# sshaoshuai/PointRCNN

Hardware: AMD Instinct MI355X
Metric: KITTI frames/sec, RPN inference end-to-end (16384 pts/frame, bs32 per GPU) (higher is better)
Workload: dtype f32 via split-bf16x6 MFMA (every fp32 operand cut exactly into 3 bf16 pieces, 6 bf16 MFMA products per fp32 product, fp32 accumulate: fp32-grade, measured error 2.9e-7 of sum|x||w| vs 3.0e-7 for the fp32-MFMA kernel; hoisted grouped layers on the split kernel too, unhoisted grouped first layers (xyz; 1 GPU; Full RPN PointNet++ backbone (4 SA-MSG + 4 FP) + cls/reg heads, tools/cfgs/default.yaml, 16384 pts/frame, batch 32 per GPU, random-init weights, eval-mode BN; frames_per_gpu=32, npoints=16384, parallelism=frames sharded, dp1, launch=hipGraph replay, streams=20, hw_queues=4, proposal_layer=normal, clouds=uniform, group_dedup=True, roi_dedup=True

## Files before the change

### include/prcnn_pointops.h

```cpp
#ifndef PRCNN_POINTOPS_H
#define PRCNN_POINTOPS_H

#include <stddef.h>
#include <stdint.h>

#ifdef __cplusplus
extern "C" {
#endif

typedef void* prcnn_stream_t;

#define PRCNN_OK 0
#define PRCNN_EINVAL (-1)
#define PRCNN_EHIP (-2)
#define PRCNN_EUNSUPPORTED (-3)

int prcnn_abi_version(void);
const char* prcnn_last_error(void);
const char* prcnn_build_id(void);
int prcnn_switches_reload(void);
int prcnn_switch_get(const char* name, int* set, long* num);


int prcnn_fps(const float* xyz, int B, int N, int npoint, float* tmp, int32_t* idx, prcnn_stream_t stream);

int prcnn_fps_status(void);

#define PRCNN_FPS_ORDER_CANONICAL 0
#define PRCNN_FPS_ORDER_UPSTREAM 1
int prcnn_fps_order(const float* xyz, int B, int N, int npoint, int order, float* tmp, int32_t* idx, prcnn_stream_t stream);

#define PRCNN_ARITH_CANONICAL 0
#define PRCNN_ARITH_UPSTREAM 1
int prcnn_fps_mode(const float* xyz, int B, int N, int npoint, int order, int arith, float* tmp, int32_t* idx, prcnn_stream_t stream);
int prcnn_ball_query_arith(const float* xyz, const float* new_xyz, int B, int N, int M, float radius, int nsample, int arith,
                           int32_t* idx, prcnn_stream_t stream);
int prcnn_three_nn_arith(const float* unknown, const float* known, int B, int n, int m, int arith, float* dist2, int32_t* idx,
                         prcnn_stream_t stream);

int prcnn_gather(const float* feat, const int32_t* idx, int B, int C, int N, int M, float* out, prcnn_stream_t stream);
int prcnn_gather_grad(const float* grad_out, const int32_t* idx, int B, int C, int N, int M, float* grad_feat,
                      prcnn_stream_t stream);

int prcnn_gather_rows(const float* in_cl, int ld_in, const int32_t* idx, int B, int N, int M, int C, float* out,
                      prcnn_stream_t stream);

int prcnn_ball_query(const float* xyz, const float* new_xyz, int B, int N, int M, float radius, int nsample,
                     int32_t* idx, prcnn_stream_t stream);
int prcnn_ball_query2(const float* xyz, const float* new_xyz, int B, int N, int M, float radius_a, int nsample_a,
                      int32_t* idx_a, float radius_b, int nsample_b, int32_t* idx_b, prcnn_stream_t stream);

int prcnn_group(const float* feat, const int32_t* idx, int B, int C, int N, int M, int nsample, float* out,
                prcnn_stream_t stream);
int prcnn_group_grad(const float* grad_out, const int32_t* idx, int B, int C, int N, int M, int nsample,
                     float* grad_feat, prcnn_stream_t stream);

int prcnn_three_nn(const float* unknown, const float* known, int B, int n, int m, float* dist2, int32_t* idx,
// ... 272 lines not shown
```

### pointrcnn_amd/_cabi.py

```python
import contextlib
import ctypes
import os

from . import build as _build

_P = ctypes.c_void_p
_I = ctypes.c_int
_F = ctypes.c_float
_L = ctypes.c_int64
_Z = ctypes.c_size_t
_D = ctypes.c_double



class TrainSrc(ctypes.Structure):
    _fields_ = [("mode", _I), ("rows", _L), ("K", _I),
                ("in_", _P), ("ld_in", _I), ("pro_scale", _P), ("pro_shift", _P),
                ("xyz", _P), ("new_xyz", _P), ("idx", _P), ("feat", _P), ("ld_feat", _I),
                ("B", _I), ("N", _I), ("M", _I), ("ns", _I), ("C", _I),
                ("known", _P), ("idx3", _P), ("w3", _P), ("skip", _P), ("ld_known", _I), ("ld_skip", _I),
                ("n", _I), ("m", _I), ("C2", _I), ("C1", _I),
                ("mult", _P), ("rows_dev", _P), ("norm_rows", _L), ("seg_off", _P), ("seg_cnt", _P), ("row_grp", _P), ("groups", _I)]


class TrainLayer(ctypes.Structure):
    _fields_ = [("Nout", _I), ("W", _P), ("gamma", _P), ("beta", _P), ("eps", _F), ("momentum", _F),
                ("running_mean", _P), ("running_var", _P), ("y", _P), ("cst", _P), ("ld_c", _I), ("wpack", _P), ("wpack_t", _P),
                ("dW", _P), ("dgamma", _P), ("dbeta", _P)]


class RpnLossCfg(ctypes.Structure):
    _fields_ = [("loc_scope", _D), ("loc_bin_size", _D), ("mean_size", _D * 3), ("gamma", _D), ("alpha", _D), ("loss_weight", _D * 2),
                ("num_head_bin", _I), ("xz_fine", _I), ("y_by_bin", _I), ("ry_fine", _I), ("loss_cls", _I), ("has_alpha", _I)]


class RcnnLossCfg(ctypes.Structure):
    _fields_ = [("loc_scope", _D), ("loc_bin_size", _D), ("loc_y_scope", _D), ("loc_y_bin_size", _D), ("mean_size", _D * 3), ("gamma", _D),
                ("alpha", _D), ("num_head_bin", _I), ("y_by_bin", _I), ("size_res_on_roi", _I), ("loss_cls", _I), ("has_alpha", _I)]


REQUIRED_ABI = 12

SIGNATURES = {
    "prcnn_abi_version": (_I, []),
    "prcnn_last_error": (ctypes.c_char_p, []),
    "prcnn_build_id": (ctypes.c_char_p, []),
    "prcnn_switches_reload": (_I, []),
    "prcnn_switch_get": (_I, [ctypes.c_char_p, ctypes.POINTER(_I), ctypes.POINTER(ctypes.c_long)]),
    "prcnn_fps": (_I, [_P, _I, _I, _I, _P, _P, _P]),
    "prcnn_fps_status": (_I, []),
    "prcnn_fps_order": (_I, [_P, _I, _I, _I, _I, _P, _P, _P]),
    "prcnn_fps_mode": (_I, [_P, _I, _I, _I, _I, _I, _P, _P, _P]),
    "prcnn_ball_query_arith": (_I, [_P, _P, _I, _I, _I, _F, _I, _I, _P, _P]),
    "prcnn_three_nn_arith": (_I, [_P, _P, _I, _I, _I, _I, _P, _P, _P]),
    "prcnn_rpn_labels": (_I, [_P, _P, _P, _I, _I, _I, _F, _P, _P, _P]),
    "prcnn_gt_aug_edit": (_I, [_P, _P, _P, _P, _P, _F, _P, _P, _P, _I, _I, _I, _I, _P, _P, _P, _P, _P]),
    "prcnn_corner_iou3d": (_I, [_P, _I, _P, _I, _P, _P, _P]),
    "prcnn_gt_aug_sample": (_I, [_P, _P, _P, _I, _I, _P, _P, _P, _I, _P, _I, _P, _I, _P, _P, _I, _I, ctypes.c_uint32,
                                 _P, _P, _P, _P, _P, _P, _P, _P]),
    "prcnn_host_pts_in_boxes3d": (_I, [_P, _P, _L, _L, _P]),
    "prcnn_host_roipool3d": (_I, [_P, _P, _P, _L, _L, _L, _L, _P, _P, _P]),
    "prcnn_gather": (_I, [_P, _P, _I, _I, _I, _I, _P, _P]),
    "prcnn_gather_grad": (_I, [_P, _P, _I, _I, _I, _I, _P, _P]),
    "prcnn_gather_rows": (_I, [_P, _I, _P, _I, _I, _I, _I, _P, _P]),
    "prcnn_ball_query": (_I, [_P, _P, _I, _I, _I, _F, _I, _P, _P]),
    "prcnn_ball_query2": (_I, [_P, _P, _I, _I, _I, _F, _I, _P, _F, _I, _P, _P]),
    "prcnn_group": (_I, [_P, _P, _I, _I, _I, _I, _I, _P, _P]),
    "prcnn_group_grad": (_I, [_P, _P, _I, _I, _I, _I, _I, _P, _P]),
    "prcnn_three_nn": (_I, [_P, _P, _I, _I, _I, _P, _P, _P, _P]),
    "prcnn_three_interp": (_I, [_P, _P, _P, _I, _I, _I, _I, _P, _P]),
    "prcnn_three_interp_grad": (_I, [_P, _P, _P, _I, _I, _I, _I, _P, _P, _P]),
    "prcnn_wpack_floats": (_Z, [_I, _I]),
    "prcnn_pack_weight": (_I, [_P, _I, _I, _I, _P, _P]),
    "prcnn_mlp_rows": (_I, [_P, _I, _L, _I, _P, _P, _I, _I, _P, _I, _I, _I, _P, _I, _P, _I, _P]),
    "prcnn_mlp_group": (_I, [_P, _P, _P, _P, _I, _I, _I, _I, _I, _I, _P, _P, _P, _P, _I, _I, _P, _I, _I, _I, _P, _P]),
    "prcnn_mlp_group_split": (_I, [_P, _P, _P, _P, _I, _I, _I, _I, _I, _I, _P, _P, _P, _P, _I, _P, _I, _I, _P, _I, _I, _I, _P, _P]),
    "prcnn_mlp_interp": (_I, [_P, _I, _P, _P, _P, _I, _I, _I, _I, _I, _I, _P, _P, _P, _I, _I, _P, _I, _I, _P]),
    "prcnn_mlp_rows_addinterp": (_I, [_P, _I, _I, _P, _P, _I, _I, _P, _I, _P, _P, _I, _I, _I, _P, _I, _I, _P]),
    "prcnn_wsplit_bytes": (_Z, [_I, _I]),
    "prcnn_pack_weight_split": (_I, [_P, _I, _I, _I, _P, _P]),
    "prcnn_mlp_chain_interp_split": (_I, [_P, _I, _P, _P, _I, _I, _I, _I, _P, _P, _P, _P, _I, _I, _I, _P, _I, _I, _P]),
    "prcnn_mlp_chain_rows_split": (_I, [_P, _I, _L, _I, _P, _P, _P, _P, _P, _I, _P, _I, _I, _P]),
# ... 146 lines not shown
```

### pointrcnn_amd/csrc/fps.hip

```cpp
#include "lds_sort.h"
#include "switches.h"

typedef float f32x2 __attribute__((ext_vector_type(2)));
template <int PPT> struct fvec_t { typedef float type __attribute__((ext_vector_type(PPT))); };
template <> struct fvec_t<1> { typedef float type __attribute__((ext_vector_type(2))); };

#define FPS_DPP_MAX(v, ctrl) asm volatile("s_nop 1\n\tv_max_i32_dpp %0, %0, %0 " ctrl : "+v"(v))

__device__ __forceinline__ int wave_max_i32_fused(int v) {
    FPS_DPP_MAX(v, "row_shr:1 row_mask:0xf bank_mask:0xf");
    FPS_DPP_MAX(v, "row_shr:2 row_mask:0xf bank_mask:0xf");
    FPS_DPP_MAX(v, "row_shr:4 row_mask:0xf bank_mask:0xf");
    FPS_DPP_MAX(v, "row_shr:8 row_mask:0xf bank_mask:0xf");
    FPS_DPP_MAX(v, "row_bcast:15 row_mask:0xa bank_mask:0xf");
    FPS_DPP_MAX(v, "row_bcast:31 row_mask:0xc bank_mask:0xf");
    asm volatile("s_nop 1");
    return __builtin_amdgcn_readlane(v, 63);
}
__device__ __forceinline__ int row0_max_i32_fused(int v) {
    FPS_DPP_MAX(v, "row_shr:1 row_mask:0xf bank_mask:0xf");
    FPS_DPP_MAX(v, "row_shr:2 row_mask:0xf bank_mask:0xf");
    FPS_DPP_MAX(v, "row_shr:4 row_mask:0xf bank_mask:0xf");
    FPS_DPP_MAX(v, "row_shr:8 row_mask:0xf bank_mask:0xf");
    asm volatile("s_nop 1");
// ... 76 lines not shown
                     : [best] "v"(best), [p0] "v"(pt[0]), [p1] "v"(pt[1]), [p2] "v"(pt[2]), [p3] "v"(pt[3])
                     : "vcc");
        eqbits = acc;
        return t;
    }
};

#define FPS_EQ2(pa, pb) "v_cmp_eq_f32_e64 %[sa], " pa ", %[best]\n\tv_cmp_eq_f32_e64 %[sb], " pb ", %[best]\n\t"
#define FPS_AC2 "v_addc_co_u32_e64 %[a0], vcc, %[a0], %[a0], %[sa]\n\tv_addc_co_u32_e64 %[a1], vcc, %[a1], %[a1], %[sb]\n\t"
template <class V> __device__ __forceinline__ int wave_max_eq2_16(const V& pt, float best, unsigned& eqbits) {
    int t; unsigned a0, a1; unsigned long long sa, sb, sc, sd;
    asm volatile("v_mov_b32 %[t], %[best]\n\tv_mov_b32 %[a0], 0\n\tv_mov_b32 %[a1], 0\n\t"
                 FPS_EQ2("%[p15]", "%[p7]") FPS_D1 FPS_AC2
                 FPS_EQ2("%[p14]", "%[p6]") FPS_D2 FPS_AC2
                 FPS_EQ2("%[p13]", "%[p5]") FPS_D3 FPS_AC2
                 FPS_EQ2("%[p12]", "%[p4]") FPS_D4 FPS_AC2
                 FPS_EQ2("%[p11]", "%[p3]") FPS_D5 FPS_AC2
                 FPS_EQ2("%[p10]", "%[p2]") FPS_D6 FPS_AC2
                 FPS_EQ2("%[p9]", "%[p1]")
                 "v_cmp_eq_f32_e64 %[sc], %[p8], %[best]\n\tv_cmp_eq_f32_e64 %[sd], %[p0], %[best]\n\t"
                 FPS_AC2
                 "v_addc_co_u32_e64 %[a0], vcc, %[a0], %[a0], %[sc]\n\tv_addc_co_u32_e64 %[a1], vcc, %[a1], %[a1], %[sd]\n\t"
                 : [t] "=&v"(t), [a0] "=&v"(a0), [a1] "=&v"(a1), [sa] "=&s"(sa), [sb] "=&s"(sb), [sc] "=&s"(sc), [sd] "=&s"(sd)
                 : [best] "v"(best), [p0] "v"(pt[0]), [p1] "v"(pt[1]), [p2] "v"(pt[2]), [p3] "v"(pt[3]), [p4] "v"(pt[4]), [p5] "v"(pt[5]),
                   [p6] "v"(pt[6]), [p7] "v"(pt[7]), [p8] "v"(pt[8]), [p9] "v"(pt[9]), [p10] "v"(pt[10]), [p11] "v"(pt[11]),
                   [p12] "v"(pt[12]), [p13] "v"(pt[13]), [p14] "v"(pt[14]), [p15] "v"(pt[15])
                 : "vcc");
    eqbits = (a0 << 8) | a1;
    return t;
}

template <int BLOCK, int PPT>
__global__ __launch_bounds__(BLOCK) void fps_reg_kernel(const float* __restrict__ xyz, int N, int npoint,
                                                        int32_t* __restrict__ idx_out) {
    constexpr int NW = BLOCK / 64;
    typedef typename fvec_t<PPT>::type fvec;
    __shared__ float slot[2][NW][8];

    const int b = blockIdx.x;
    const int tid = threadIdx.x;
    const int lane = tid & 63;
    const int wave = tid >> 6;
    const float* __restrict__ p = xyz + (size_t)b * N * 3;
    int32_t* __restrict__ out = idx_out + (size_t)b * npoint;

    fvec px, py, pz, pt;
#pragma unroll
    for (int i = 0; i < PPT; i++) {
        int k = tid * PPT + i;
        bool ok = k < N;
        px[i] = ok ? p[k * 3 + 0] : 0.f;
        py[i] = ok ? p[k * 3 + 1] : 0.f;
        pz[i] = ok ? p[k * 3 + 2] : 0.f;
        pt[i] = ok ? 1e10f : -1.0f;
    }
    if (tid == 0 && npoint > 0) out[0] = 0;
    float x0 = p[0], y0 = p[1], z0 = p[2];

    for (int j = 1; j < npoint; j++) {
        float best = -2.0f;
        if (PPT >= 2) {
            const f32x2 qx = {x0, x0}, qy = {y0, y0}, qz = {z0, z0};
#pragma unroll
            for (int i = 0; i + 1 < PPT; i += 2) {
                f32x2 dx = (f32x2){px[i], px[i + 1]} - qx;
                f32x2 dy = (f32x2){py[i], py[i + 1]} - qy;
                f32x2 dz = (f32x2){pz[i], pz[i + 1]} - qz;
// ... 31 lines not shown
            }
            __syncthreads();
            const float* r = slot[j & 1][lane < NW ? lane : 0];
            int v = lane < NW ? __float_as_int(r[0]) : (int)0x80000000;
            int id = __float_as_int(r[1]);
            float rx = r[2], ry = r[3], rz = r[4];
            const int gmax = row0_max_i32_fused(v);
            const int wwin = __builtin_ctzll(__ballot(v == gmax));
            gidx = __builtin_amdgcn_readlane(id, wwin);
            x0 = __int_as_float(__builtin_amdgcn_readlane(__float_as_int(rx), wwin));
            y0 = __int_as_float(__builtin_amdgcn_readlane(__float_as_int(ry), wwin));
            z0 = __int_as_float(__builtin_amdgcn_readlane(__float_as_int(rz), wwin));
        }
        if (tid == 0) out[j] = gidx;
    }
}

#define FPS_BIG 1.0e18f
#ifndef FPS_V
#define FPS_V 6
#endif
#ifndef FPS_PAIR_ASM
#define FPS_PAIR_ASM 1
#endif

__device__ __forceinline__ unsigned morton_spread6(unsigned v) {
    v &= 0x3fu;
    v = (v | (v << 8)) & 0x0000300fu;
    v = (v | (v << 4)) & 0x000030c3u;
    v = (v | (v << 2)) & 0x00009249u;
    return v;
}

__global__ __launch_bounds__(1024) void fps_sort_kernel(const float* __restrict__ xyz, int N, int NP, int32_t* __restrict__ perm) {
    extern __shared__ unsigned keys[];
    __shared__ float red[6][16];
    const int b = blockIdx.x, tid = threadIdx.x, lane = tid & 63, wave = tid >> 6, nw = blockDim.x >> 6;
    const float* __restrict__ p = xyz + (size_t)b * N * 3;
    float lo[3] = {FPS_BIG, FPS_BIG, FPS_BIG}, hi[3] = {-FPS_BIG, -FPS_BIG, -FPS_BIG};
    for (int k = tid; k < N; k += blockDim.x)
#pragma unroll
        for (int a = 0; a < 3; a++) { float v = p[k * 3 + a]; lo[a] = fminf(lo[a], v); hi[a] = fmaxf(hi[a], v); }
#pragma unroll
    for (int a = 0; a < 3; a++) {
        for (int o = 32; o > 0; o >>= 1) { lo[a] = fminf(lo[a], __shfl_xor(lo[a], o)); hi[a] = fmaxf(hi[a], __shfl_xor(hi[a], o)); }
        if (lane == 0) { red[a][wave] = lo[a]; red[3 + a][wave] = hi[a]; }
    }
    __syncthreads();
    float scale[3];
#pragma unroll
    for (int a = 0; a < 3; a++) {
        float l = red[a][0], h = red[3 + a][0];
        for (int w = 1; w < nw; w++) { l = fminf(l, red[a][w]); h = fmaxf(h, red[3 + a][w]); }
        lo[a] = l;
        scale[a] = (h > l) ? 63.0f / (h - l) : 0.f;
    }
    unsigned v[16];
    if (tid * 16 < NP) {
#pragma unroll
        for (int e = 0; e < 16; e++) {
            const int k = tid * 16 + e;
            unsigned key = ~0u;
            if (k < N) {
                unsigned qx = (unsigned)((p[k * 3 + 0] - lo[0]) * scale[0]);
                unsigned qy = (unsigned)((p[k * 3 + 1] - lo[1]) * scale[1]);
                unsigned qz = (unsigned)((p[k * 3 + 2] - lo[2]) * scale[2]);
                unsigned m = (morton_spread6(qx) << 2) | (morton_spread6(qz) << 1) | morton_spread6(qy);
// ... 50 lines not shown
}
__device__ __forceinline__ void fps_xt_publish(unsigned (*xt)[64], int cb, int wave, const fps_cand_t& c) {
    unsigned* t = xt[cb];
    t[wave] = __float_as_uint(c.x); t[16 + wave] = __float_as_uint(c.y); t[32 + wave] = __float_as_uint(c.z);
    asm volatile("ds_max_u64 %0, %1 offset:192" : : "v"((unsigned)(size_t)&t[0]), "v"(c.key) : "memory");
    if (wave == 0) *(unsigned long long*)&xt[cb == 2 ? 0 : cb + 1][48] = 0ULL;
}
__device__ __forceinline__ int fps_xt_collect(unsigned (*xt)[64], int cb, int lane, float& x0, float& y0, float& z0, int& wl) {
    const int tv = (int)xt[cb][lane];
    const unsigned klo = (unsigned)__builtin_amdgcn_readlane(tv, 48);
    wl = (int)(klo & 15u);
    x0 = __int_as_float(__builtin_amdgcn_readlane(tv, wl));
    y0 = __int_as_float(__builtin_amdgcn_readlane(tv, wl | 16));
    z0 = __int_as_float(__builtin_amdgcn_readlane(tv, wl | 32));
    return (int)(0xFFFFFFFu - (klo >> 4));
}

#ifdef PRCNN_FPS_TIMING
__device__ unsigned long long prcnn_fps_dbg[16 * 8 + 16 + 16 * 16];
PRCNN_API int prcnn_fps_timing_read(unsigned long long* host_out) {
    return hipMemcpyFromSymbol(host_out, HIP_SYMBOL(prcnn_fps_dbg), sizeof(prcnn_fps_dbg)) == hipSuccess ? 0 : -1;
}
#define FPS_T(...) __VA_ARGS__
#ifndef PRCNN_FPS_TIMING_WAVE
#define PRCNN_FPS_TIMING_WAVE -1
#endif
#define FPS_NOW(w) ((PRCNN_FPS_TIMING_WAVE < 0 || (w) == PRCNN_FPS_TIMING_WAVE) ? __builtin_readcyclecounter() : 0ULL)
#else
#define FPS_T(...)
#endif

template <int PPT>
__global__ __launch_bounds__(1024) void fps_pruned_kernel(const float* __restrict__ xyz, const int32_t* __restrict__ perm,
                                                          int N, int npoint, int32_t* __restrict__ idx_out) {
    constexpr int BLOCK = 1024, NW = 16;
    typedef typename fvec_t<PPT>::type fvec;
    FPS_XT_DECL;
    extern __shared__ int s_po[];
    __builtin_amdgcn_s_setprio(2);

    const int b = blockIdx.x, tid = threadIdx.x, lane = tid & 63, wave = tid >> 6;
    const int wave_u = __builtin_amdgcn_readfirstlane(wave);
    const float* __restrict__ p = xyz + (size_t)b * N * 3;
    const int32_t* __restrict__ pm = perm + (size_t)b * N;
    int32_t* __restrict__ out = idx_out + (size_t)b * npoint;

    fvec px, py, pz, pt;
    float lox = FPS_BIG, loy = FPS_BIG, loz = FPS_BIG, hix = -FPS_BIG, hiy = -FPS_BIG, hiz = -FPS_BIG;
#pragma unroll
    for (int i = 0; i < PPT; i++) {
        int s = tid * PPT + i;
        bool ok = s < N;
        int o = ok ? pm[s] : 0x7fffffff;
        s_po[i * BLOCK + tid] = o;
        px[i] = ok ? p[o * 3 + 0] : 0.f;
        py[i] = ok ? p[o * 3 + 1] : 0.f;
        pz[i] = ok ? p[o * 3 + 2] : 0.f;
        pt[i] = ok ? 1e10f : -1.0f;
        if (ok) {
            lox = fminf(lox, px[i]); hix = fmaxf(hix, px[i]);
            loy = fminf(loy, py[i]); hiy = fmaxf(hiy, py[i]);
            loz = fminf(loz, pz[i]); hiz = fmaxf(hiz, pz[i]);
        }
    }
    lox = wave_min_f32_fused(lox); loy = wave_min_f32_fused(loy); loz = wave_min_f32_fused(loz);
    hix = wave_max_f32_fused(hix); hiy = wave_max_f32_fused(hiy); hiz = wave_max_f32_fused(hiz);

// ... 78 lines not shown
                cy = __int_as_float(__builtin_amdgcn_readlane(__float_as_int(by), owner));
                cz = __int_as_float(__builtin_amdgcn_readlane(__float_as_int(bz), owner));
            }
            cval = wmaxf;
            first = false;
            fps_cand_set(cand, wave, cx, cy, cz, cval, corig);
            FPS_T(t_u4 += __builtin_readcyclecounter() - u3;)
            }
            __builtin_amdgcn_s_setprio(2);
        }
#if FPS_V & 2
        else __builtin_amdgcn_s_setprio(2);
#endif
        FPS_T(unsigned long long t1 = __builtin_readcyclecounter(); t_upd += t1 - t0; n_upd += update ? 1 : 0;)
        if (lane == 0) fps_xt_publish(xt, cb, wave, cand);
        __syncthreads();
        FPS_T(unsigned long long t2 = __builtin_readcyclecounter(); t_wait += t2 - t1;)
        int wwin;
        const int gorig = fps_xt_collect(xt, cb, lane, x0, y0, z0, wwin);
#if FPS_V & 2
        if ((unsigned)(wave_u - wwin + 1) <= 2u) __builtin_amdgcn_s_setprio(3);
#endif
        wprev = wwin;
        cb = cb == 2 ? 0 : cb + 1;
        if (tid == 0) out[j] = gorig;
        FPS_T(t0 = __builtin_readcyclecounter(); t_red += t0 - t2;)
    }
    FPS_T(if (b == 0 && lane == 0) { unsigned long long* d = prcnn_fps_dbg + wave * 8; d[0] = t_upd; d[1] = t_wait; d[2] = t_red; d[3] = n_upd;
                                     d[4] = __builtin_readcyclecounter() - t_begin; d[5] = t_u1; d[6] = t_u2; d[7] = t_u3; prcnn_fps_dbg[128 + wave] = t_u4; })
}

template <int PPT, int NW>
__global__ __launch_bounds__(NW * 64) void fps_slot_kernel(const float* __restrict__ xyz, const int32_t* __restrict__ perm,
                                                          int N, int npoint, int32_t* __restrict__ idx_out) {
    constexpr int BLOCK = NW * 64;
    typedef typename fvec_t<PPT>::type fvec;
    FPS_XT_DECL;
    extern __shared__ int s_po[];
    __builtin_amdgcn_s_setprio(2);

    const int b = blockIdx.x, tid = threadIdx.x, lane = tid & 63, wave = tid >> 6;
    const int wave_u = __builtin_amdgcn_readfirstlane(wave);
    const float* __restrict__ p = xyz + (size_t)b * N * 3;
    const int32_t* __restrict__ pm = perm + (size_t)b * N;
    int32_t* __restrict__ out = idx_out + (size_t)b * npoint;

    fvec px, py, pz, pt;
    float lox = FPS_BIG, loy = FPS_BIG, loz = FPS_BIG, hix = -FPS_BIG, hiy = -FPS_BIG, hiz = -FPS_BIG;
#pragma unroll
    for (int i = 0; i < PPT; i++) {
        int s = (wave * PPT + i) * 64 + lane;
        bool ok = s < N;
        int o = ok ? pm[s] : 0x7fffffff;
        s_po[i * BLOCK + tid] = o;
        px[i] = ok ? p[o * 3 + 0] : 0.f;
        py[i] = ok ? p[o * 3 + 1] : 0.f;
        pz[i] = ok ? p[o * 3 + 2] : 0.f;
        pt[i] = ok ? 1e10f : -1.0f;
        if (ok) {
            lox = fminf(lox, px[i]); hix = fmaxf(hix, px[i]);
            loy = fminf(loy, py[i]); hiy = fmaxf(hiy, py[i]);
            loz = fminf(loz, pz[i]); hiz = fmaxf(hiz, pz[i]);
        }
    }
    lox = wave_min_f32_fused(lox); loy = wave_min_f32_fused(loy); loz = wave_min_f32_fused(loz);
    hix = wave_max_f32_fused(hix); hiy = wave_max_f32_fused(hiy); hiz = wave_max_f32_fused(hiz);

// ... 136 lines not shown
        }
#if FPS_V & 2
        else __builtin_amdgcn_s_setprio(2);
#endif
        FPS_T(unsigned long long q4 = FPS_NOW(wave);)
        if (lane == 0) fps_xt_publish(xt, cb, wave, cand);
        __syncthreads();
        FPS_T(unsigned long long q5 = FPS_NOW(wave); q_pub += q5 - q4;)
        int wwin;
        const int gorig = fps_xt_collect(xt, cb, lane, x0, y0, z0, wwin);
#if FPS_V & 2
        if ((unsigned)(wave_u - wwin + 1) <= 2u) __builtin_amdgcn_s_setprio(3);
#endif
        wprev = wwin;
        cb = cb == 2 ? 0 : cb + 1;
        if (tid == 0) out[j] = gorig;
        FPS_T(q0 = FPS_NOW(wave); q_coll += q0 - q5;)
    }
    FPS_T(if (b == 0 && lane == 0) { unsigned long long* d = prcnn_fps_dbg + 144 + wave * 16; d[0] = q_test; d[1] = q_dist; d[2] = q_max; d[3] = q_search; d[4] = q_pub;
                                     d[5] = q_coll; d[6] = q_nupd; d[7] = q_npair; d[8] = FPS_NOW(wave) - q_begin; })
}

struct fps_bcand_t { float x, y, z, v, s; unsigned orig, mask; unsigned long long key; };
__device__ __forceinline__ void fps_bcand_set(fps_bcand_t& c, int wave, float cx, float cy, float cz, float cval, float csec, int corig, unsigned cmask) {
    const unsigned hi = (unsigned)__float_as_int(cval) ^ 0x80000000u;
    const unsigned o = (unsigned)min(corig, 0xFFFFFFF);
    c.x = cx; c.y = cy; c.z = cz; c.v = cval; c.s = csec; c.orig = o; c.mask = cmask; c.key = ((unsigned long long)hi << 32) | ((0xFFFFFFFu - o) << 4) | (unsigned)wave;
    asm volatile("" : "+v"(c.x), "+v"(c.y), "+v"(c.z), "+v"(c.v), "+v"(c.s), "+v"(c.orig), "+v"(c.mask), "+v"(c.key));
}
#define FPS_BT_WORDS 160

template <int PPT, int NW>
__global__ __launch_bounds__(NW * 64) void fps_batch_kernel(const float* __restrict__ xyz, const int32_t* __restrict__ perm,
                                                           int N, int npoint, int32_t* __restrict__ idx_out) {
    static_assert(NW == 16 && PPT == 16, "rows of 16 lanes = the 16 waves; 8 pair boxes");
    constexpr int BLOCK = NW * 64;
    typedef typename fvec_t<PPT>::type fvec;
    typedef float f32x4 __attribute__((ext_vector_type(4)));
    typedef unsigned u32x4 __attribute__((ext_vector_type(4)));
    __shared__ __attribute__((aligned(256))) unsigned xt[3][FPS_BT_WORDS];
    __shared__ __attribute__((aligned(32))) float wbox[16][8];
    extern __shared__ int s_po[];
    __builtin_amdgcn_s_setprio(2);

    const int b = blockIdx.x, tid = threadIdx.x, lane = tid & 63, wave = tid >> 6, l15 = lane & 15;
    const int wave_u = __builtin_amdgcn_readfirstlane(wave);
    const float* __restrict__ p = xyz + (size_t)b * N * 3;
    const int32_t* __restrict__ pm = perm + (size_t)b * N;
    int32_t* __restrict__ out = idx_out + (size_t)b * npoint;

    fvec px, py, pz, pt;
    float lox = FPS_BIG, loy = FPS_BIG, loz = FPS_BIG, hix = -FPS_BIG, hiy = -FPS_BIG, hiz = -FPS_BIG;
#pragma unroll
    for (int i = 0; i < PPT; i++) {
        int s = (wave * PPT + i) * 64 + lane;
        bool ok = s < N;
        int o = ok ? pm[s] : 0x7fffffff;
        s_po[i * BLOCK + tid] = o;
        px[i] = ok ? p[o * 3 + 0] : 0.f;
        py[i] = ok ? p[o * 3 + 1] : 0.f;
        pz[i] = ok ? p[o * 3 + 2] : 0.f;
        pt[i] = ok ? 1e10f : -1.0f;
        if (ok) {
            lox = fminf(lox, px[i]); hix = fmaxf(hix, px[i]);
            loy = fminf(loy, py[i]); hiy = fmaxf(hiy, py[i]);
            loz = fminf(loz, pz[i]); hiz = fmaxf(hiz, pz[i]);
        }
// ... 294 lines not shown
    __shared__ int sval[2][NW], sidx[2][NW];
    const int b = blockIdx.x, tid = threadIdx.x, lane = tid & 63, wave = tid >> 6;
    const float* __restrict__ p = xyz + (size_t)b * N * 3;
    float* __restrict__ t = tmp + (size_t)b * N;
    int32_t* __restrict__ out = idx_out + (size_t)b * npoint;
    for (int k = tid; k < N; k += 1024) t[k] = 1e10f;
    if (tid == 0 && npoint > 0) out[0] = 0;
    int old = 0;
    for (int j = 1; j < npoint; j++) {
        float x0 = p[old * 3], y0 = p[old * 3 + 1], z0 = p[old * 3 + 2];
        float best = -2.0f;
        int bk = 0x7fffffff;
        for (int k = tid; k < N; k += 1024) {
            float d = sqdist3(p[k * 3], p[k * 3 + 1], p[k * 3 + 2], x0, y0, z0);
            float v = t[k];
            v = d < v ? d : v;
            t[k] = v;
            if (v > best) { best = v; bk = k; }
        }
        int vb = __float_as_int(best);
        int wmax = wave_max_i32(vb);
        int widx = wave_min_i32(vb == wmax ? bk : 0x7fffffff);
        if (lane == 0) { sval[j & 1][wave] = wmax; sidx[j & 1][wave] = widx; }
        __syncthreads();
        int v = lane < NW ? sval[j & 1][lane] : (int)0x80000000;
        int id = lane < NW ? sidx[j & 1][lane] : 0x7fffffff;
        int gmax = row0_max_i32(v);
        old = row0_min_i32(v == gmax ? id : 0x7fffffff);
        if (tid == 0) out[j] = old;
    }
}

template <int BLOCK, int PPT>
static void launch_fps(const float* xyz, int B, int N, int npoint, int32_t* idx, hipStream_t s) {
    hipLaunchKernelGGL((fps_reg_kernel<BLOCK, PPT>), dim3(B), dim3(BLOCK), 0, s, xyz, N, npoint, idx);
}

static int* fps_timeout_word() {
    static int* word = [] {
        int* w = nullptr;
        if (hipHostMalloc((void**)&w, sizeof(int), hipHostMallocMapped) != hipSuccess) { (void)hipGetLastError(); return (int*)nullptr; }
        *w = 0;
        return w;
    }();
    return word;
}

PRCNN_API int prcnn_fps_status(void) {
    int* w = fps_timeout_word();
    if (w && __atomic_exchange_n(w, 0, __ATOMIC_RELAXED) != 0)
        return prcnn_fail(PRCNN_EHIP, "prcnn_fps: a multi-workgroup launch (N > 16384) gave up waiting for a partner slice; "
                                      "its output holds -1 indices (were all ceil(N/16384) workgroups of a frame able to become resident?)");
    return PRCNN_OK;
}

PRCNN_API int prcnn_fps(const float* xyz, int B, int N, int npoint, float* tmp, int32_t* idx, prcnn_stream_t stream) {
    PRCNN_REQUIRE(B >= 0 && N > 0 && npoint >= 0, "prcnn_fps: bad shape B=%d N=%d npoint=%d", B, N, npoint);
    PRCNN_REQUIRE(npoint <= N, "prcnn_fps: npoint %d > N %d", npoint, N);
    if (B == 0 || npoint == 0) return PRCNN_OK;
    PRCNN_REQUIRE(xyz && idx, "prcnn_fps: null pointer");
    hipStream_t s = (hipStream_t)stream;
    if (tmp && N > 2048 && N <= 16384) {
        int NP = 1;
        while (NP < N) NP <<= 1;
        int32_t* perm = reinterpret_cast<int32_t*>(tmp);
        static PrcnnLdsLimit sort_attr;
        if (!sort_attr.raise((const void*)fps_sort_kernel, 80 * 1024))
            return prcnn_fail(PRCNN_EHIP, "prcnn_fps: cannot raise the dynamic LDS limit of the sort kernel");
        const int sort_threads = NP / 16 < 64 ? 64 : NP / 16;
        hipLaunchKernelGGL(fps_sort_kernel, dim3(B), dim3(sort_threads), lds_sort_bytes(NP, sizeof(unsigned)), s, xyz, N, NP, perm);
        PRCNN_LAUNCH_CHECK("prcnn_fps(sort)");
        static PrcnnLdsLimit pruned_attr;
        if (!pruned_attr.raise((const void*)fps_pruned_kernel<16>, 16 * 4096))
            return prcnn_fail(PRCNN_EHIP, "prcnn_fps: cannot raise the dynamic LDS limit of the pruned kernel");
        const bool slots = sw_enabled(SW_FPS_SLOTS);
        static PrcnnLdsLimit slot_attr;
        if (slots && N > 8192 && !slot_attr.raise((const void*)fps_slot_kernel<16, 16>, 16 * 4096))
            return prcnn_fail(PRCNN_EHIP, "prcnn_fps: cannot raise the dynamic LDS limit of the slot kernel");
        const bool batch = sw_opt_in(SW_FPS_BATCH);
        static PrcnnLdsLimit batch_attr;
        if (slots && batch && N > 8192 && !batch_attr.raise((const void*)fps_batch_kernel<16, 16>, 16 * 4096))
            return prcnn_fail(PRCNN_EHIP, "prcnn_fps: cannot raise the dynamic LDS limit of the batch kernel");
        if (slots && batch && N > 8192) hipLaunchKernelGGL((fps_batch_kernel<16, 16>), dim3(B), dim3(1024), 16 * 4096, s, xyz, perm, N, npoint, idx);
        else if (slots && N > 8192) hipLaunchKernelGGL((fps_slot_kernel<16, 16>), dim3(B), dim3(1024), 16 * 4096, s, xyz, perm, N, npoint, idx);
        else if (N <= 4096) hipLaunchKernelGGL((fps_pruned_kernel<4>), dim3(B), dim3(1024), 4 * 4096, s, xyz, perm, N, npoint, idx);
        else if (N <= 8192) hipLaunchKernelGGL((fps_pruned_kernel<8>), dim3(B), dim3(1024), 8 * 4096, s, xyz, perm, N, npoint, idx);
        else hipLaunchKernelGGL((fps_pruned_kernel<16>), dim3(B), dim3(1024), 16 * 4096, s, xyz, perm, N, npoint, idx);
    }
    else if (N <= 64) launch_fps<64, 1>(xyz, B, N, npoint, idx, s);
    else if (N <= 128) launch_fps<64, 2>(xyz, B, N, npoint, idx, s);
    else if (N <= 256) launch_fps<64, 4>(xyz, B, N, npoint, idx, s);
    else if (N <= 512) launch_fps<64, 8>(xyz, B, N, npoint, idx, s);
    else if (N <= 1024) launch_fps<64, 16>(xyz, B, N, npoint, idx, s);
    else if (N <= 2048) launch_fps<256, 8>(xyz, B, N, npoint, idx, s);
    else if (N <= 4096) launch_fps<256, 16>(xyz, B, N, npoint, idx, s);
    else if (N <= 8192) launch_fps<1024, 8>(xyz, B, N, npoint, idx, s);
    else if (N <= 16384) launch_fps<1024, 16>(xyz, B, N, npoint, idx, s);
    else {
        PRCNN_REQUIRE(tmp, "prcnn_fps: N=%d > 16384 needs the (B,N) tmp buffer", N);
        const int S = prcnn_divup(N, FPS_MULTI_SLICE);
        const bool use_mem = sw_present(SW_FPS_MEM);
        if (!use_mem && S <= FPS_MULTI_MAX_SPLIT && ((uintptr_t)tmp & 7) == 0) {
            const size_t slot_bytes = (size_t)B * 2 * S * 5 * sizeof(unsigned long long);
            if (prcnn_fill_words(tmp, 0xFFFFFFFFu, slot_bytes / 4, s) != hipSuccess) return prcnn_fail(PRCNN_EHIP, "prcnn_fps: cannot clear the exchange slots");
            if (int st = prcnn_fps_status()) return st;
            hipLaunchKernelGGL(fps_multi_kernel, dim3(B * S), dim3(1024), 0, s, xyz, N, npoint, S, reinterpret_cast<unsigned long long*>(tmp), idx,
                               fps_timeout_word());
        } else {
            hipLaunchKernelGGL(fps_mem_kernel, dim3(B), dim3(1024), 0, s, xyz, N, npoint, tmp, idx);
        }
    }
    PRCNN_LAUNCH_CHECK("prcnn_fps");
    return PRCNN_OK;
}

__global__ __launch_bounds__(1024) void fps_upstream_order_kernel(const float* __restrict__ xyz, int N, int npoint, int T,
                                                                  float* __restrict__ tmp, int32_t* __restrict__ idx_out) {
    constexpr int NWMAX = 16;
    __shared__ int sval[2][NWMAX], stid[2][NWMAX], sidx[2][NWMAX];
    const int b = blockIdx.x, tid = threadIdx.x, lane = tid & 63, wave = tid >> 6;
    const int nw = (blockDim.x + 63) >> 6;
    const float* __restrict__ p = xyz + (size_t)b * N * 3;
    float* __restrict__ t = tmp + (size_t)b * N;
    int32_t* __restrict__ out = idx_out + (size_t)b * npoint;
    for (int k = tid; k < N; k += blockDim.x) t[k] = 1e10f;
    if (tid == 0 && npoint > 0) out[0] = 0;
    __syncthreads();
    int old = 0;
    for (int j = 1; j < npoint; j++) {
        const float x0 = p[old * 3], y0 = p[old * 3 + 1], z0 = p[old * 3 + 2];
        float best = -2.0f;
        int bk = 0x7fffffff;
        if (tid < T) {
            for (int k = tid; k < N; k += T) {
                const float d = sqdist3(p[k * 3], p[k * 3 + 1], p[k * 3 + 2], x0, y0, z0);
                float v = t[k];
                v = d < v ? d : v;
                t[k] = v;
                if (v > best) { best = v; bk = k; }
            }
        }
        const int vb = __float_as_int(best);
        const int wmax = wave_max_i32(vb);
        const int wtid = wave_min_i32(vb == wmax ? tid : 0x7fffffff);
        const int wk = __shfl(bk, wtid & 63);
        if (lane == 0) { sval[j & 1][wave] = wmax; stid[j & 1][wave] = wtid; sidx[j & 1][wave] = wk; }
// ... 26 lines not shown
```

### pointrcnn_amd/ops.py

```python
import ctypes
import math
import os
import threading

import torch

from . import _cabi

_INT = torch.int32
_F32 = torch.float32
FPS_PRUNED = os.environ.get("PRCNN_FPS_PRUNED", "1") == "1"


def _stream():
    return torch.cuda.current_stream().cuda_stream


def _chk(t, name, dtype=_F32, ndim=None):
    if not isinstance(t, torch.Tensor):
        raise TypeError("%s must be a torch.Tensor" % name)
    if not t.is_cuda:
        raise RuntimeError("%s must be a CUDA(HIP) tensor: the HIP kernels are the only implementation" % name)
    if t.dtype != dtype:
        raise RuntimeError("%s must have dtype %s, got %s" % (name, dtype, t.dtype))
    if not t.is_contiguous():
        raise RuntimeError("%s must be contiguous" % name)
    if ndim is not None and t.dim() != ndim:
        raise RuntimeError("%s must have %d dims, got shape %s" % (name, ndim, tuple(t.shape)))
    return t


def _p(t):
    return None if t is None else t.data_ptr()


def furthest_point_sample(xyz, npoint, order="canonical"):
    _chk(xyz, "xyz", ndim=3)
    B, N, _ = xyz.shape
    idx = torch.empty((B, npoint), dtype=_INT, device=xyz.device)
    if order != "canonical":
        if order != "upstream":
            raise ValueError("furthest_point_sample: order must be 'canonical' or 'upstream'")
        tmp = torch.empty((B, N), dtype=_F32, device=xyz.device)
        _cabi.check(_cabi.lib().prcnn_fps_order(_p(xyz), B, N, npoint, 1, _p(tmp), _p(idx), _stream()), "prcnn_fps_order")
        return idx
    tmp = torch.empty((B, N), dtype=_F32, device=xyz.device) if (N > 16384 or (N > 2048 and FPS_PRUNED)) else None
    L = _cabi.lib()
    _cabi.check(L.prcnn_fps(_p(xyz), B, N, npoint, _p(tmp), _p(idx), _stream()), "prcnn_fps")
    return idx


_ARITH = {"canonical": 0, "upstream": 1}
_ORDER = {"canonical": 0, "upstream": 1}


def furthest_point_sample_mode(xyz, npoint, order="canonical", arith="canonical"):
    _chk(xyz, "xyz", ndim=3)
    B, N, _ = xyz.shape
    idx = torch.empty((B, npoint), dtype=_INT, device=xyz.device)
    tmp = torch.empty((B, N), dtype=_F32, device=xyz.device)
    _cabi.check(_cabi.lib().prcnn_fps_mode(_p(xyz), B, N, npoint, _ORDER[order], _ARITH[arith], _p(tmp), _p(idx), _stream()), "prcnn_fps_mode")
    return idx


def ball_query_arith(radius, nsample, xyz, new_xyz, arith="upstream"):
    _chk(xyz, "xyz", ndim=3); _chk(new_xyz, "new_xyz", ndim=3)
    B, N, _ = xyz.shape
    M = new_xyz.shape[1]
    idx = torch.empty((B, M, nsample), dtype=_INT, device=xyz.device)
    _cabi.check(_cabi.lib().prcnn_ball_query_arith(_p(xyz), _p(new_xyz), B, N, M, float(radius), nsample, _ARITH[arith], _p(idx), _stream()),
                "prcnn_ball_query_arith")
    return idx


def three_nn_arith(unknown, known, arith="upstream"):
    _chk(unknown, "unknown", ndim=3); _chk(known, "known", ndim=3)
    B, n, _ = unknown.shape
    m = known.shape[1]
    d2 = torch.empty((B, n, 3), dtype=_F32, device=unknown.device)
    idx = torch.empty((B, n, 3), dtype=_INT, device=unknown.device)
    _cabi.check(_cabi.lib().prcnn_three_nn_arith(_p(unknown), _p(known), B, n, m, _ARITH[arith], _p(d2), _p(idx), _stream()),
                "prcnn_three_nn_arith")
    return d2, idx


def fps_status():
    _cabi.check(_cabi.lib().prcnn_fps_status(), "prcnn_fps_status")


def gather(features, idx):
    _chk(features, "features", ndim=3); _chk(idx, "idx", _INT, 2)
    B, C, N = features.shape
    M = idx.shape[1]
    out = torch.empty((B, C, M), dtype=_F32, device=features.device)
    _cabi.check(_cabi.lib().prcnn_gather(_p(features), _p(idx), B, C, N, M, _p(out), _stream()), "prcnn_gather")
    return out


def gather_grad(grad_out, idx, N):
    _chk(grad_out, "grad_out", ndim=3); _chk(idx, "idx", _INT, 2)
    B, C, M = grad_out.shape
    g = torch.zeros((B, C, N), dtype=_F32, device=grad_out.device)
    _cabi.check(_cabi.lib().prcnn_gather_grad(_p(grad_out), _p(idx), B, C, N, M, _p(g), _stream()), "prcnn_gather_grad")
    return g


def gather_rows(in_cl, idx):
    _chk(idx, "idx", _INT, 2)
    B, N, C = in_cl.shape
    M = idx.shape[1]
    out = torch.empty((B, M, C), dtype=_F32, device=in_cl.device)
    _cabi.check(_cabi.lib().prcnn_gather_rows(_p(in_cl), _row_stride(in_cl), _p(idx), B, N, M, C, _p(out), _stream()),
                "prcnn_gather_rows")
    return out


GRID_MIN_POINTS = 2048 if os.environ.get("PRCNN_GRID_SEARCH", "1") != "0" else 1 << 62
THREE_NN_GRID_MIN = int(os.environ.get("PRCNN_THREE_NN_GRID_MIN", "1024")) if GRID_MIN_POINTS < (1 << 62) else 1 << 62
DENSE_SCAN = os.environ.get("PRCNN_DENSE_SCAN", "1") != "0"
BQ_GRID_CELLS = int(os.environ.get("PRCNN_BQ_GRID_CELLS", "128"))


class Grid:

    def __init__(self, xyz, min_cell=0.0, cells_per_axis=64):
        _chk(xyz, "xyz", ndim=3)
        self.B, self.N = xyz.shape[0], xyz.shape[1]
        L = _cabi.lib()
        nbytes = L.prcnn_grid_bytes(self.B, self.N)
        self.buf = torch.empty((max(nbytes, 16),), dtype=torch.uint8, device=xyz.device)
        _cabi.check(L.prcnn_grid_build(_p(xyz), self.B, self.N, float(min_cell), int(cells_per_axis), _p(self.buf), nbytes, _stream()),
                    "prcnn_grid_build")


def ball_query_grid(grid, new_xyz, radius_a, nsample_a, radius_b=0.0, nsample_b=0, xyz=None):
    _chk(new_xyz, "new_xyz", ndim=3)
    B, M = new_xyz.shape[0], new_xyz.shape[1]
    if B != grid.B:
        raise ValueError("ball_query_grid: %d frames of centroids vs %d frames in the grid" % (B, grid.B))
    ia = torch.empty((B, M, nsample_a), dtype=_INT, device=new_xyz.device)
    ib = torch.empty((B, M, nsample_b), dtype=_INT, device=new_xyz.device) if nsample_b else None
    _cabi.check(_cabi.lib().prcnn_ball_query2_grid(_p(grid.buf), _p(xyz), _p(new_xyz), B, grid.N, M, float(radius_a), nsample_a, _p(ia),
                                                   float(radius_b), nsample_b, _p(ib), _stream()), "prcnn_ball_query2_grid")
    return (ia, ib) if nsample_b else ia


# ... 983 lines not shown
```

Before: 13570 frames/s.

## Skip nested FPS when input points are a gathered prefix of prior FPS

Records on the gathered xyz tensor that it came from an earlier farthest-point-sampling result. Later FPS calls on that tensor launch a cheap prefix kernel instead. The kernel checks validity (finite-range coordinates, no padding duplicates of index 0), writes the identity prefix, and sets per-batch skip words so the heavy FPS kernels exit early. This relies on FPS of an FPS-ordered subset returning its own prefix, which removes the sequential FPS cost of the later SA levels. It adds one small kernel launch, attribute bookkeeping on tensors, and a tie-breaking edge case. The path is disabled for inference-mode tensors.

```diff
diff --git a/include/prcnn_pointops.h b/include/prcnn_pointops.h
--- a/include/prcnn_pointops.h
+++ b/include/prcnn_pointops.h
@@ -23,6 +23,9 @@
 
 
 int prcnn_fps(const float* xyz, int B, int N, int npoint, float* tmp, int32_t* idx, prcnn_stream_t stream);
+
+int prcnn_fps_nested(const float* xyz, const int32_t* prev_idx, int B, int N, int npoint, float* tmp, int32_t* idx, int32_t* skip,
+                     prcnn_stream_t stream);
 
 int prcnn_fps_status(void);
 
diff --git a/pointrcnn_amd/_cabi.py b/pointrcnn_amd/_cabi.py
--- a/pointrcnn_amd/_cabi.py
+++ b/pointrcnn_amd/_cabi.py
@@ -48,6 +48,7 @@
     "prcnn_switches_reload": (_I, []),
     "prcnn_switch_get": (_I, [ctypes.c_char_p, ctypes.POINTER(_I), ctypes.POINTER(ctypes.c_long)]),
     "prcnn_fps": (_I, [_P, _I, _I, _I, _P, _P, _P]),
+    "prcnn_fps_nested": (_I, [_P, _P, _I, _I, _I, _P, _P, _P, _P]),
     "prcnn_fps_status": (_I, []),
     "prcnn_fps_order": (_I, [_P, _I, _I, _I, _I, _P, _P, _P]),
     "prcnn_fps_mode": (_I, [_P, _I, _I, _I, _I, _I, _P, _P, _P]),
diff --git a/pointrcnn_amd/csrc/fps.hip b/pointrcnn_amd/csrc/fps.hip
--- a/pointrcnn_amd/csrc/fps.hip
+++ b/pointrcnn_amd/csrc/fps.hip
@@ -132,7 +132,8 @@
 
 template <int BLOCK, int PPT>
 __global__ __launch_bounds__(BLOCK) void fps_reg_kernel(const float* __restrict__ xyz, int N, int npoint,
-                                                        int32_t* __restrict__ idx_out) {
+                                                        int32_t* __restrict__ idx_out, const int32_t* __restrict__ skip) {
+    if (skip && skip[blockIdx.x]) return;
     constexpr int NW = BLOCK / 64;
     typedef typename fvec_t<PPT>::type fvec;
     __shared__ float slot[2][NW][8];
@@ -230,7 +231,9 @@
     return v;
 }
 
-__global__ __launch_bounds__(1024) void fps_sort_kernel(const float* __restrict__ xyz, int N, int NP, int32_t* __restrict__ perm) {
+__global__ __launch_bounds__(1024) void fps_sort_kernel(const float* __restrict__ xyz, int N, int NP, int32_t* __restrict__ perm,
+                                                        const int32_t* __restrict__ skip) {
+    if (skip && skip[blockIdx.x]) return;
     extern __shared__ unsigned keys[];
     __shared__ float red[6][16];
     const int b = blockIdx.x, tid = threadIdx.x, lane = tid & 63, wave = tid >> 6, nw = blockDim.x >> 6;
@@ -347,7 +350,8 @@
 
 template <int PPT>
 __global__ __launch_bounds__(1024) void fps_pruned_kernel(const float* __restrict__ xyz, const int32_t* __restrict__ perm,
-                                                          int N, int npoint, int32_t* __restrict__ idx_out) {
+                                                          int N, int npoint, int32_t* __restrict__ idx_out, const int32_t* __restrict__ skip) {
+    if (skip && skip[blockIdx.x]) return;
     constexpr int BLOCK = 1024, NW = 16;
     typedef typename fvec_t<PPT>::type fvec;
     FPS_XT_DECL;
@@ -492,7 +496,8 @@
 
 template <int PPT, int NW>
 __global__ __launch_bounds__(NW * 64) void fps_slot_kernel(const float* __restrict__ xyz, const int32_t* __restrict__ perm,
-                                                          int N, int npoint, int32_t* __restrict__ idx_out) {
+                                                          int N, int npoint, int32_t* __restrict__ idx_out, const int32_t* __restrict__ skip) {
+    if (skip && skip[blockIdx.x]) return;
     constexpr int BLOCK = NW * 64;
     typedef typename fvec_t<PPT>::type fvec;
     FPS_XT_DECL;
@@ -695,7 +700,8 @@
 
 template <int PPT, int NW>
 __global__ __launch_bounds__(NW * 64) void fps_batch_kernel(const float* __restrict__ xyz, const int32_t* __restrict__ perm,
-                                                           int N, int npoint, int32_t* __restrict__ idx_out) {
+                                                           int N, int npoint, int32_t* __restrict__ idx_out, const int32_t* __restrict__ skip) {
+    if (skip && skip[blockIdx.x]) return;
     static_assert(NW == 16 && PPT == 16, "rows of 16 lanes = the 16 waves; 8 pair boxes");
     constexpr int BLOCK = NW * 64;
     typedef typename fvec_t<PPT>::type fvec;
@@ -1056,8 +1062,8 @@
 }
 
 template <int BLOCK, int PPT>
-static void launch_fps(const float* xyz, int B, int N, int npoint, int32_t* idx, hipStream_t s) {
-    hipLaunchKernelGGL((fps_reg_kernel<BLOCK, PPT>), dim3(B), dim3(BLOCK), 0, s, xyz, N, npoint, idx);
+static void launch_fps(const float* xyz, int B, int N, int npoint, int32_t* idx, const int32_t* skip, hipStream_t s) {
+    hipLaunchKernelGGL((fps_reg_kernel<BLOCK, PPT>), dim3(B), dim3(BLOCK), 0, s, xyz, N, npoint, idx, skip);
 }
 
 static int* fps_timeout_word() {
@@ -1078,12 +1084,22 @@
     return PRCNN_OK;
 }
 
-PRCNN_API int prcnn_fps(const float* xyz, int B, int N, int npoint, float* tmp, int32_t* idx, prcnn_stream_t stream) {
-    PRCNN_REQUIRE(B >= 0 && N > 0 && npoint >= 0, "prcnn_fps: bad shape B=%d N=%d npoint=%d", B, N, npoint);
-    PRCNN_REQUIRE(npoint <= N, "prcnn_fps: npoint %d > N %d", npoint, N);
-    if (B == 0 || npoint == 0) return PRCNN_OK;
-    PRCNN_REQUIRE(xyz && idx, "prcnn_fps: null pointer");
-    hipStream_t s = (hipStream_t)stream;
+__global__ __launch_bounds__(256) void fps_prefix_kernel(const float* __restrict__ xyz, const int32_t* __restrict__ prev_idx, int N, int npoint,
+                                                         int32_t* __restrict__ idx_out, int32_t* __restrict__ skip) {
+    const int b = blockIdx.x, tid = threadIdx.x;
+    const float* __restrict__ p = xyz + (size_t)b * N * 3;
+    const int32_t* __restrict__ pi = prev_idx + (size_t)b * N;
+    int32_t* __restrict__ out = idx_out + (size_t)b * npoint;
+    bool ok = true;
+    for (int k = tid; k < 3 * N; k += 256) ok &= fabsf(p[k]) < 1e4f;
+    for (int j = 1 + tid; j < npoint; j += 256) ok &= pi[j] != 0;
+    const int pass = __syncthreads_and(ok) ? 1 : 0;
+    if (pass)
+        for (int j = tid; j < npoint; j += 256) out[j] = j;
+    if (tid == 0) skip[b] = pass;
+}
+
+static int fps_dispatch(const float* xyz, int B, int N, int npoint, float* tmp, int32_t* idx, const int32_t* skip, hipStream_t s) {
     if (tmp && N > 2048 && N <= 16384) {
         int NP = 1;
         while (NP < N) NP <<= 1;
@@ -1092,7 +1108,7 @@
         if (!sort_attr.raise((const void*)fps_sort_kernel, 80 * 1024))
             return prcnn_fail(PRCNN_EHIP, "prcnn_fps: cannot raise the dynamic LDS limit of the sort kernel");
         const int sort_threads = NP / 16 < 64 ? 64 : NP / 16;
-        hipLaunchKernelGGL(fps_sort_kernel, dim3(B), dim3(sort_threads), lds_sort_bytes(NP, sizeof(unsigned)), s, xyz, N, NP, perm);
+        hipLaunchKernelGGL(fps_sort_kernel, dim3(B), dim3(sort_threads), lds_sort_bytes(NP, sizeof(unsigned)), s, xyz, N, NP, perm, skip);
         PRCNN_LAUNCH_CHECK("prcnn_fps(sort)");
         static PrcnnLdsLimit pruned_attr;
         if (!pruned_attr.raise((const void*)fps_pruned_kernel<16>, 16 * 4096))
@@ -1105,23 +1121,24 @@
         static PrcnnLdsLimit batch_attr;
         if (slots && batch && N > 8192 && !batch_attr.raise((const void*)fps_batch_kernel<16, 16>, 16 * 4096))
             return prcnn_fail(PRCNN_EHIP, "prcnn_fps: cannot raise the dynamic LDS limit of the batch kernel");
-        if (slots && batch && N > 8192) hipLaunchKernelGGL((fps_batch_kernel<16, 16>), dim3(B), dim3(1024), 16 * 4096, s, xyz, perm, N, npoint, idx);
-        else if (slots && N > 8192) hipLaunchKernelGGL((fps_slot_kernel<16, 16>), dim3(B), dim3(1024), 16 * 4096, s, xyz, perm, N, npoint, idx);
-        else if (N <= 4096) hipLaunchKernelGGL((fps_pruned_kernel<4>), dim3(B), dim3(1024), 4 * 4096, s, xyz, perm, N, npoint, idx);
-        else if (N <= 8192) hipLaunchKernelGGL((fps_pruned_kernel<8>), dim3(B), dim3(1024), 8 * 4096, s, xyz, perm, N, npoint, idx);
-        else hipLaunchKernelGGL((fps_pruned_kernel<16>), dim3(B), dim3(1024), 16 * 4096, s, xyz, perm, N, npoint, idx);
-    }
-    else if (N <= 64) launch_fps<64, 1>(xyz, B, N, npoint, idx, s);
-    else if (N <= 128) launch_fps<64, 2>(xyz, B, N, npoint, idx, s);
-    else if (N <= 256) launch_fps<64, 4>(xyz, B, N, npoint, idx, s);
-    else if (N <= 512) launch_fps<64, 8>(xyz, B, N, npoint, idx, s);
-    else if (N <= 1024) launch_fps<64, 16>(xyz, B, N, npoint, idx, s);
-    else if (N <= 2048) launch_fps<256, 8>(xyz, B, N, npoint, idx, s);
-    else if (N <= 4096) launch_fps<256, 16>(xyz, B, N, npoint, idx, s);
-    else if (N <= 8192) launch_fps<1024, 8>(xyz, B, N, npoint, idx, s);
-    else if (N <= 16384) launch_fps<1024, 16>(xyz, B, N, npoint, idx, s);
+        if (slots && batch && N > 8192) hipLaunchKernelGGL((fps_batch_kernel<16, 16>), dim3(B), dim3(1024), 16 * 4096, s, xyz, perm, N, npoint, idx, skip);
+        else if (slots && N > 8192) hipLaunchKernelGGL((fps_slot_kernel<16, 16>), dim3(B), dim3(1024), 16 * 4096, s, xyz, perm, N, npoint, idx, skip);
+        else if (N <= 4096) hipLaunchKernelGGL((fps_pruned_kernel<4>), dim3(B), dim3(1024), 4 * 4096, s, xyz, perm, N, npoint, idx, skip);
+        else if (N <= 8192) hipLaunchKernelGGL((fps_pruned_kernel<8>), dim3(B), dim3(1024), 8 * 4096, s, xyz, perm, N, npoint, idx, skip);
+        else hipLaunchKernelGGL((fps_pruned_kernel<16>), dim3(B), dim3(1024), 16 * 4096, s, xyz, perm, N, npoint, idx, skip);
+    }
+    else if (N <= 64) launch_fps<64, 1>(xyz, B, N, npoint, idx, skip, s);
+    else if (N <= 128) launch_fps<64, 2>(xyz, B, N, npoint, idx, skip, s);
+    else if (N <= 256) launch_fps<64, 4>(xyz, B, N, npoint, idx, skip, s);
+    else if (N <= 512) launch_fps<64, 8>(xyz, B, N, npoint, idx, skip, s);
+    else if (N <= 1024) launch_fps<64, 16>(xyz, B, N, npoint, idx, skip, s);
+    else if (N <= 2048) launch_fps<256, 8>(xyz, B, N, npoint, idx, skip, s);
+    else if (N <= 4096) launch_fps<256, 16>(xyz, B, N, npoint, idx, skip, s);
+    else if (N <= 8192) launch_fps<1024, 8>(xyz, B, N, npoint, idx, skip, s);
+    else if (N <= 16384) launch_fps<1024, 16>(xyz, B, N, npoint, idx, skip, s);
     else {
         PRCNN_REQUIRE(tmp, "prcnn_fps: N=%d > 16384 needs the (B,N) tmp buffer", N);
+        PRCNN_REQUIRE(!skip, "prcnn_fps: the multi-workgroup kernels (N=%d > 16384) take no skip words", N);
         const int S = prcnn_divup(N, FPS_MULTI_SLICE);
         const bool use_mem = sw_present(SW_FPS_MEM);
         if (!use_mem && S <= FPS_MULTI_MAX_SPLIT && ((uintptr_t)tmp & 7) == 0) {
@@ -1136,6 +1153,27 @@
     }
     PRCNN_LAUNCH_CHECK("prcnn_fps");
     return PRCNN_OK;
+}
+
+PRCNN_API int prcnn_fps(const float* xyz, int B, int N, int npoint, float* tmp, int32_t* idx, prcnn_stream_t stream) {
+    PRCNN_REQUIRE(B >= 0 && N > 0 && npoint >= 0, "prcnn_fps: bad shape B=%d N=%d npoint=%d", B, N, npoint);
+    PRCNN_REQUIRE(npoint <= N, "prcnn_fps: npoint %d > N %d", npoint, N);
+    if (B == 0 || npoint == 0) return PRCNN_OK;
+    PRCNN_REQUIRE(xyz && idx, "prcnn_fps: null pointer");
+    return fps_dispatch(xyz, B, N, npoint, tmp, idx, nullptr, (hipStream_t)stream);
+}
+
+PRCNN_API int prcnn_fps_nested(const float* xyz, const int32_t* prev_idx, int B, int N, int npoint, float* tmp, int32_t* idx, int32_t* skip,
+                               prcnn_stream_t stream) {
+    PRCNN_REQUIRE(B >= 0 && N > 0 && npoint >= 0, "prcnn_fps_nested: bad shape B=%d N=%d npoint=%d", B, N, npoint);
+    PRCNN_REQUIRE(npoint <= N, "prcnn_fps_nested: npoint %d > N %d", npoint, N);
+    PRCNN_REQUIRE(N <= 16384, "prcnn_fps_nested: N=%d > 16384 (call prcnn_fps)", N);
+    if (B == 0 || npoint == 0) return PRCNN_OK;
+    PRCNN_REQUIRE(xyz && prev_idx && idx && skip, "prcnn_fps_nested: null pointer");
+    hipStream_t s = (hipStream_t)stream;
+    hipLaunchKernelGGL(fps_prefix_kernel, dim3(B), dim3(256), 0, s, xyz, prev_idx, N, npoint, idx, skip);
+    PRCNN_LAUNCH_CHECK("prcnn_fps_nested(prefix)");
+    return fps_dispatch(xyz, B, N, npoint, tmp, idx, skip, s);
 }
 
 __global__ __launch_bounds__(1024) void fps_upstream_order_kernel(const float* __restrict__ xyz, int N, int npoint, int T,
diff --git a/pointrcnn_amd/ops.py b/pointrcnn_amd/ops.py
--- a/pointrcnn_amd/ops.py
+++ b/pointrcnn_amd/ops.py
@@ -2,6 +2,7 @@
 import math
 import os
 import threading
+import weakref
 
 import torch
 
@@ -10,6 +11,7 @@
 _INT = torch.int32
 _F32 = torch.float32
 FPS_PRUNED = os.environ.get("PRCNN_FPS_PRUNED", "1") == "1"
+FPS_NESTED = os.environ.get("PRCNN_FPS_NESTED", "1") == "1"
 
 
 def _stream():
@@ -34,6 +36,14 @@
     return None if t is None else t.data_ptr()
 
 
+def _tensor_key(t):
+    return (t.data_ptr(), tuple(t.shape), tuple(t.stride()), t._version)
+
+
+def _hintable(*tensors):
+    return FPS_NESTED and not any(t.is_inference() for t in tensors)
+
+
 def furthest_point_sample(xyz, npoint, order="canonical"):
     _chk(xyz, "xyz", ndim=3)
     B, N, _ = xyz.shape
@@ -46,7 +56,19 @@
         return idx
     tmp = torch.empty((B, N), dtype=_F32, device=xyz.device) if (N > 16384 or (N > 2048 and FPS_PRUNED)) else None
     L = _cabi.lib()
-    _cabi.check(L.prcnn_fps(_p(xyz), B, N, npoint, _p(tmp), _p(idx), _stream()), "prcnn_fps")
+    parent = getattr(xyz, "_prcnn_fps_parent", None) if _hintable(xyz) else None
+    if parent is not None:
+        prev_idx, prev_version, key = parent
+        if not (_hintable(prev_idx) and key == _tensor_key(xyz) and prev_idx._version == prev_version and prev_idx.device == xyz.device
+                and tuple(prev_idx.shape) == (B, N) and npoint <= N <= 16384):
+            parent = None
+    if parent is not None:
+        skip = torch.empty((B,), dtype=_INT, device=xyz.device)
+        _cabi.check(L.prcnn_fps_nested(_p(xyz), _p(prev_idx), B, N, npoint, _p(tmp), _p(idx), _p(skip), _stream()), "prcnn_fps_nested")
+    else:
+        _cabi.check(L.prcnn_fps(_p(xyz), B, N, npoint, _p(tmp), _p(idx), _stream()), "prcnn_fps")
+    if _hintable(xyz, idx):
+        idx._prcnn_fps_src = (weakref.ref(xyz), _tensor_key(xyz), idx._version)
     return idx
 
 
@@ -112,6 +134,9 @@
     out = torch.empty((B, M, C), dtype=_F32, device=in_cl.device)
     _cabi.check(_cabi.lib().prcnn_gather_rows(_p(in_cl), _row_stride(in_cl), _p(idx), B, N, M, C, _p(out), _stream()),
                 "prcnn_gather_rows")
+    src = getattr(idx, "_prcnn_fps_src", None) if (C == 3 and _hintable(in_cl, idx, out)) else None
+    if src is not None and src[0]() is in_cl and src[1] == _tensor_key(in_cl) and src[2] == idx._version:
+        out._prcnn_fps_parent = (idx, idx._version, _tensor_key(out))
     return out
 
 
```

Measured after the change: 14090 frames/s (median of 6 runs). +3.8%, better.
